# VladGavra98/SERL

Measured on AMD Instinct MI355X. Metric: env-steps/sec (whole node), pop-rollout eval, pop=50 nominal per GPU, higher is better.
Workload: dtype f64

## Files before the change

### serl_amd/csrc/citation_step_dev.h

```cpp
#if !defined(CIT_MODEL) || !defined(CIT_DERIV) || !defined(CIT_STEP)
#error "define CIT_MODEL, CIT_DERIV and CIT_STEP"
#endif
#ifndef CIT_STEP_ATTR
#define CIT_STEP_ATTR __noinline__
#endif
static __device__ CIT_STEP_ATTR void CIT_STEP(CitCtx *gc, const double *cmd_in, double *out_arg)
{
  CitCtx lc;
#ifdef CIT_CMD_IN_MEMORY
  double y[19], f[6][19], out[12];
#else
  double y[19], f[6][19], cmd[10], out[12];
#endif
  for (int i = 0; i < 19; ++i) { lc.X[i] = gc->X[i]; y[i] = lc.X[i]; }
#ifdef CIT_DW_IN_MEMORY
  lc.dwm = gc->DW;
#else
  for (int i = 0; i < 29; ++i) lc.DW[i] = gc->DW[i];
#endif
  for (int i = 0; i < 4; ++i) lc.IW[i] = gc->IW[i];
#ifndef CIT_Y_IS_STATE
  for (int i = 0; i < 12; ++i) lc.Y[i] = gc->Y[i];
#endif
#ifdef CIT_USE_HINTS
  for (int i = 0; i < (CIT_USE_HINTS + 5) / 6; ++i) lc.hint[i] = gc->hint[i];
#endif
#ifdef CIT_CMD_IN_MEMORY
  const double *cmd = cmd_in;
#else
  for (int i = 0; i < 10; ++i) cmd[i] = cmd_in[i];
#endif
  lc.t = gc->t; lc.stop_time = gc->stop_time; lc.dt = gc->dt; lc.tick = gc->tick;
  lc.ro = gc->ro; lc.t3 = gc->t3; lc.err = gc->err; lc.bslot = gc->bslot;
  const double t0 = lc.t, h = lc.dt;
  for (int s = 0; s < 6; ++s) {
    if (s > 0) {
      double hB[6];
      for (int j = 0; j < s; ++j) hB[j] = cit_ode5_B[s - 1][j] * h;
      for (int i = 0; i < 19; ++i) {
        double acc = f[0][i] * hB[0];
        for (int j = 1; j < s; ++j) acc = acc + f[j][i] * hB[j];
        lc.X[i] = acc + y[i];
      }
      lc.t = (s == 5) ? lc.stop_time : (s == 1 ? hB[0] + t0 : h * cit_ode5_A[s - 1] + t0);
    }
    lc.major = (s == 0) ? 1 : 0;
#ifndef CIT_NO_AXES
    cit_axes_prepare(&lc.ax, lc.X[4], lc.X[5], lc.X[6], lc.X[7], lc.X[8]);
#endif
    CIT_MODEL(&lc, cmd, out);
    CIT_DERIV(&lc, f[s]);
  }
  {
    double hB[6];
    for (int j = 0; j < 6; ++j) hB[j] = cit_ode5_B[5][j] * h;
    for (int i = 0; i < 19; ++i) {
      double acc = f[0][i] * hB[0];
      for (int j = 1; j < 6; ++j) acc = acc + f[j][i] * hB[j];
      gc->X[i] = acc + y[i];
    }
  }
#ifndef CIT_DW_IN_MEMORY
  for (int i = 0; i < 29; ++i) gc->DW[i] = lc.DW[i];
#endif
  for (int i = 0; i < 4; ++i) gc->IW[i] = lc.IW[i];
#ifdef CIT_Y_IS_STATE
  for (int i = 0; i < 12; ++i) { gc->Y[i] = y[i]; out_arg[i] = y[i]; }
#else
  for (int i = 0; i < 12; ++i) { gc->Y[i] = lc.Y[i]; out_arg[i] = lc.Y[i]; }
#endif
#ifdef CIT_USE_HINTS
  for (int i = 0; i < (CIT_USE_HINTS + 5) / 6; ++i) gc->hint[i] = lc.hint[i];
#endif
  gc->major = 1;
  gc->err = lc.err;
  gc->tick = lc.tick + 1;
  gc->stop_time = lc.stop_time;
  gc->t = lc.stop_time;
}
#undef CIT_MODEL
#undef CIT_DERIV
#undef CIT_STEP
#undef CIT_USE_HINTS
#undef CIT_Y_IS_STATE
#undef CIT_DW_IN_MEMORY
#undef CIT_CMD_IN_MEMORY
```

### serl_amd/csrc/family_lane.hip

```cpp
#include "citation_dev.h"
#include "rollout_device.h"
#include "serl_variant.h"
#ifdef SERL_VENV_NOISE
#include "serl_rng.h"
#endif
#ifdef SERL_ROLLOUT_NOISE
#include "rollout_noise.h"
#endif
#define CIT_V(x) SERL_PASTE(SERL_PASTE(cit_, VARIANT), x)
#define CIT_RO_LO_W CIT_V(_RO_LO_W)
#define CIT_RO_HI_W CIT_V(_RO_HI_W)
#define RO_BASE_W CIT_V(_RO_BASE_W)

namespace bdag {
#define CIT_B_AT(i) (c->B[(i)])
#define SERL_FLAVOUR_LDS 0
#define CIT_NO_AXES 1
#ifndef CIT_CTX_FLAT
#define CIT_DWM_PTR __attribute__((address_space(5))) double *
#define CIT_CMD_PTR const __attribute__((address_space(5))) double *
#else
#define CIT_DWM_PTR double *
#define CIT_CMD_PTR const double *
#endif
#include SERL_GEN_LANE
static_assert(CIT_RO_HI_W - CIT_RO_LO_W <= CIT_RO_LDS_WORDS, "LDS table window too small");
static_assert(8 * (CIT_RO_LDS_WORDS + CIT_V(_NSLOPE)) <= 160 * 1024, "tables + interval quotients beyond the 160 KB of LDS");
#define CIT_MODEL CIT_V(_dag_model)
#define CIT_DERIV CIT_V(_dag_derivatives)
#define CIT_STEP SERL_PASTE(cit_step_, VARIANT)
#define CIT_SLOPE_DESC CIT_V(_slope_desc)
#define CIT_SLOPE_TABLES CIT_V(_NSLOPE_TABLES)
#define CIT_USE_HINTS CIT_V(_NSEARCH)
#define CIT_DW_IN_MEMORY 1
#ifdef CIT_WITH_CMD_IN_MEMORY
#define CIT_CMD_IN_MEMORY 1
#endif
#if !defined(SERL_ROLLOUT_NOISE) && !defined(SERL_LANE_GENERAL_ACTOR)
#define SERL_LANE_QUEUE 1
#endif
#define CIT_Y_IS_STATE 1
#include "citation_step_dev.h"
#include "rollout_variant.inc"
#if !defined(SERL_ROLLOUT_NOISE) && !defined(SERL_LANE_GENERAL_ACTOR)
#include "venv_variant.inc"
#endif
#undef CIT_NO_AXES
#undef CIT_B_AT
#undef SERL_FLAVOUR_LDS
}

#define SERL_V(x) SERL_PASTE(x, VARIANT)
#if defined(SERL_LANE_GENERAL_ACTOR) && defined(SERL_LANE_REGROUPED_WEIGHTS)
#ifdef SERL_ROLLOUT_NOISE
void SERL_V(serl_launch_rollout_lanegt_noise_)(const RolloutArgs &a, const serl_rollout_noise_desc &nz, int grid, hipStream_t stream) { bdag::SERL_V(serl_launch_rollout_lanegt_noise_)(a, nz, grid, stream); }
#else
void SERL_V(serl_launch_rollout_lanegt_)(const RolloutArgs &a, int grid, hipStream_t stream) { bdag::SERL_V(serl_launch_rollout_lanegt_)(a, grid, stream); }
#endif
#elif defined(SERL_LANE_GENERAL_ACTOR)
#ifdef SERL_ROLLOUT_NOISE
void SERL_V(serl_launch_rollout_laneg_noise_)(const RolloutArgs &a, const serl_rollout_noise_desc &nz, int grid, hipStream_t stream) { bdag::SERL_V(serl_launch_rollout_laneg_noise_)(a, nz, grid, stream); }
#else
void SERL_V(serl_launch_rollout_laneg_)(const RolloutArgs &a, int grid, hipStream_t stream) { bdag::SERL_V(serl_launch_rollout_laneg_)(a, grid, stream); }
#endif
#elif defined(SERL_ROLLOUT_NOISE)
void SERL_V(serl_launch_rollout_noise_)(const RolloutArgs &a, const serl_rollout_noise_desc &nz, int grid, hipStream_t stream) { bdag::SERL_V(serl_launch_rollout_noise_)(a, nz, grid, stream); }
#elif defined(SERL_VENV_NOISE)
#define SERL_VNZ(x) SERL_PASTE(SERL_PASTE(x, noise_), VARIANT)
void SERL_VNZ(serl_launch_venv_reset_)(const RolloutArgs &a, const VenvArgs &v, const serl_venv_noise_desc &nz, int grid, hipStream_t stream) { bdag::SERL_VNZ(serl_launch_venv_reset_)(a, v, nz, grid, stream); }
void SERL_VNZ(serl_launch_venv_step_auto_)(const RolloutArgs &a, const VenvArgs &v, const serl_venv_auto_desc &au, const serl_venv_noise_desc &nz, int grid, hipStream_t stream) { bdag::SERL_VNZ(serl_launch_venv_step_auto_)(a, v, au, nz, grid, stream); }
void SERL_VNZ(serl_launch_venv_rollout_)(const RolloutArgs &a, const VenvArgs &v, const serl_venv_auto_desc &au, const serl_venv_rollout_desc &rd, const serl_venv_noise_desc &nz, int grid, hipStream_t stream) { bdag::SERL_VNZ(serl_launch_venv_rollout_)(a, v, au, rd, nz, grid, stream); }
void SERL_VNZ(serl_launch_venv_rollout_general_)(const RolloutArgs &a, const VenvArgs &v, const serl_venv_auto_desc &au, const serl_venv_rollout_desc &rd, const serl_venv_noise_desc &nz, int grid, hipStream_t stream) { bdag::SERL_VNZ(serl_launch_venv_rollout_general_)(a, v, au, rd, nz, grid, stream); }
#else
void SERL_V(serl_launch_rollout_)(const RolloutArgs &a, int grid, hipStream_t stream) { bdag::SERL_V(serl_launch_rollout_)(a, grid, stream); }
void SERL_V(serl_launch_rollout_laneq_)(const RolloutArgs &a, int grid, hipStream_t stream) { bdag::SERL_V(serl_launch_rollout_laneq_)(a, grid, stream); }

void SERL_V(serl_launch_dyn_)(const RolloutArgs &a, const double *cmds, double *states, int T, int grid, hipStream_t stream)
{
  bdag::SERL_V(serl_launch_dyn_)(a, cmds, states, T, grid, stream);
}

void SERL_V(serl_launch_venv_reset_)(const RolloutArgs &a, const VenvArgs &v, int grid, hipStream_t stream) { bdag::SERL_V(serl_launch_venv_reset_)(a, v, grid, stream); }
void SERL_V(serl_launch_venv_step_)(const RolloutArgs &a, const VenvArgs &v, int grid, hipStream_t stream) { bdag::SERL_V(serl_launch_venv_step_)(a, v, grid, stream); }
void SERL_V(serl_launch_venv_step_auto_)(const RolloutArgs &a, const VenvArgs &v, const serl_venv_auto_desc &au, int grid, hipStream_t stream) { bdag::SERL_V(serl_launch_venv_step_auto_)(a, v, au, grid, stream); }
void SERL_V(serl_launch_venv_rollout_)(const RolloutArgs &a, const VenvArgs &v, const serl_venv_auto_desc &au, const serl_venv_rollout_desc &rd, int grid, hipStream_t stream) { bdag::SERL_V(serl_launch_venv_rollout_)(a, v, au, rd, grid, stream); }
void SERL_V(serl_launch_venv_rollout_general_)(const RolloutArgs &a, const VenvArgs &v, const serl_venv_auto_desc &au, const serl_venv_rollout_desc &rd, int grid, hipStream_t stream) { bdag::SERL_V(serl_launch_venv_rollout_general_)(a, v, au, rd, grid, stream); }
#endif
```

### serl_amd/csrc/gen/citation_cg_timed_lane.inc

```
enum { cit_cg_timed_RO_BASE_W = 9216, cit_cg_timed_RO_LO_W = 9914, cit_cg_timed_RO_HI_W = 21883 };
enum { cit_cg_timed_NSEARCH = 47 };
enum { cit_cg_timed_NSLOPE = 8435, cit_cg_timed_NSLOPE_TABLES = 70 };
__shared__ double g_sl[cit_cg_timed_NSLOPE];
static __device__ const int cit_cg_timed_slope_desc[70][6] = {
  {1, 5091, 2, 1, 5089, 0},
  {1, 11914, 2, 1, 11912, 1},
  {1, 3085, 3, 1, 3082, 2},
  {1, 5590, 3, 1, 3088, 4},
  {1, 6444, 3, 1, 3088, 6},
  {1, 8405, 3, 1, 3088, 8},
  {1, 8408, 3, 1, 3088, 10},
  {1, 8414, 3, 1, 8411, 12},
  {1, 8414, 3, 1, 8417, 14},
  {1, 10200, 3, 1, 3088, 16},
  {2, 2594, 2, 2, 2590, 18},
  {2, 3103, 2, 2, 2590, 20},
  {2, 3131, 2, 2, 2590, 22},
  {2, 3131, 2, 2, 4115, 24},
  {2, 3135, 2, 2, 2590, 26},
  {2, 3139, 2, 2, 2590, 28},
  {2, 3143, 2, 2, 2590, 30},
  {2, 4117, 2, 2, 4115, 32},
  {2, 5577, 2, 2, 2590, 34},
  {2, 6255, 2, 2, 2590, 36},
  {2, 6261, 2, 2, 2590, 38},
  {2, 6346, 2, 2, 4115, 40},
  {2, 6350, 2, 2, 2590, 42},
  {2, 8424, 2, 2, 8420, 44},
  {2, 10213, 2, 2, 2590, 46},
  {2, 10404, 2, 2, 2590, 48},
  {2, 10498, 2, 2, 2590, 50},
  {1, 11920, 4, 1, 11916, 52},
  {1, 11907, 5, 1, 11902, 55},
  {1, 11924, 5, 1, 11902, 59},
  {1, 11896, 6, 1, 11890, 63},
  {2, 3094, 3, 3, 3088, 68},
  {2, 5581, 3, 3, 3088, 74},
  {2, 6147, 3, 3, 3088, 80},
  {2, 6435, 3, 3, 3088, 86},
  {2, 10191, 3, 3, 3088, 92},
  {2, 10314, 3, 3, 3088, 98},
  {2, 10408, 3, 3, 3088, 104},
  {1, 132, 10, 1, 122, 110},
  {1, 5593, 10, 1, 122, 119},
  {1, 10203, 10, 1, 122, 128},
  {2, 3115, 4, 4, 3107, 137},
  {2, 10298, 4, 4, 3107, 149},
  {2, 1744, 6, 6, 1732, 161},
  {2, 6174, 9, 9, 6156, 191},
  {2, 6265, 9, 9, 6156, 263},
  {2, 6354, 9, 9, 6156, 335},
  {2, 10217, 9, 9, 6156, 407},
  {2, 10323, 9, 9, 6156, 479},
  {2, 10417, 9, 9, 6156, 551},
  {2, 11614, 9, 9, 11596, 623},
  {2, 11469, 11, 11, 11447, 695},
  {2, 11721, 13, 13, 11695, 805},
  {2, 1814, 17, 17, 1780, 961},
  {2, 8428, 17, 17, 1780, 1233},
  {2, 214, 22, 22, 170, 1505},
  {2, 756, 22, 22, 734, 1967},
  {2, 1248, 22, 22, 734, 2429},
  {2, 2106, 22, 22, 734, 2891},
  {2, 2598, 22, 22, 734, 3353},
  {2, 3147, 22, 22, 170, 3815},
  {2, 3631, 22, 22, 734, 4277},
  {2, 4121, 22, 22, 734, 4739},
  {2, 4605, 22, 22, 734, 5201},
  {2, 5093, 22, 22, 734, 5663},
  {2, 5606, 22, 22, 734, 6125},
  {2, 6447, 22, 22, 170, 6587},
  {2, 6931, 22, 22, 734, 7049},
  {2, 7437, 22, 22, 7415, 7511},
  {2, 7921, 22, 22, 734, 7973},
};
static __device__ __forceinline__ double cit_table3_val(CitCtx *c, double u0, double u1, double u2)
{
  double y; cit_table3(c, &u0, &u1, &u2, &y); return y;
}
LIFT_INLINE void cit_cg_timed_dag_model(CitCtx *c, const double *cmd, double *out)
{
  (void)out;
  const double *X = c->X;
  const bool major = c->major != 0;
// ... 1338 lines not shown
```

### serl_amd/csrc/gen/citation_gust_lane.inc

```
enum { cit_gust_RO_BASE_W = 9216, cit_gust_RO_LO_W = 9914, cit_gust_RO_HI_W = 21888 };
enum { cit_gust_NSEARCH = 46 };
enum { cit_gust_NSLOPE = 8435, cit_gust_NSLOPE_TABLES = 70 };
__shared__ double g_sl[cit_gust_NSLOPE];
static __device__ const int cit_gust_slope_desc[70][6] = {
  {1, 5075, 2, 1, 5073, 0},
  {1, 11898, 2, 1, 11896, 1},
  {1, 3069, 3, 1, 3066, 2},
  {1, 5574, 3, 1, 3072, 4},
  {1, 6428, 3, 1, 3072, 6},
  {1, 8389, 3, 1, 3072, 8},
  {1, 8392, 3, 1, 3072, 10},
  {1, 8398, 3, 1, 8395, 12},
  {1, 8398, 3, 1, 8401, 14},
  {1, 10184, 3, 1, 3072, 16},
  {2, 2578, 2, 2, 2574, 18},
  {2, 3087, 2, 2, 2574, 20},
  {2, 3115, 2, 2, 2574, 22},
  {2, 3115, 2, 2, 4099, 24},
  {2, 3119, 2, 2, 2574, 26},
  {2, 3123, 2, 2, 2574, 28},
  {2, 3127, 2, 2, 2574, 30},
  {2, 4101, 2, 2, 4099, 32},
  {2, 5561, 2, 2, 2574, 34},
  {2, 6239, 2, 2, 2574, 36},
  {2, 6245, 2, 2, 2574, 38},
  {2, 6330, 2, 2, 4099, 40},
  {2, 6334, 2, 2, 2574, 42},
  {2, 8408, 2, 2, 8404, 44},
  {2, 10197, 2, 2, 2574, 46},
  {2, 10388, 2, 2, 2574, 48},
  {2, 10482, 2, 2, 2574, 50},
  {1, 11904, 4, 1, 11900, 52},
  {1, 11891, 5, 1, 11886, 55},
  {1, 11908, 5, 1, 11886, 59},
  {1, 11880, 6, 1, 11874, 63},
  {2, 3078, 3, 3, 3072, 68},
  {2, 5565, 3, 3, 3072, 74},
  {2, 6131, 3, 3, 3072, 80},
  {2, 6419, 3, 3, 3072, 86},
  {2, 10175, 3, 3, 3072, 92},
  {2, 10298, 3, 3, 3072, 98},
  {2, 10392, 3, 3, 3072, 104},
  {1, 132, 10, 1, 122, 110},
  {1, 5577, 10, 1, 122, 119},
  {1, 10187, 10, 1, 122, 128},
  {2, 3099, 4, 4, 3091, 137},
  {2, 10282, 4, 4, 3091, 149},
  {2, 1728, 6, 6, 1716, 161},
  {2, 6158, 9, 9, 6140, 191},
  {2, 6249, 9, 9, 6140, 263},
  {2, 6338, 9, 9, 6140, 335},
  {2, 10201, 9, 9, 6140, 407},
  {2, 10307, 9, 9, 6140, 479},
  {2, 10401, 9, 9, 6140, 551},
  {2, 11598, 9, 9, 11580, 623},
  {2, 11453, 11, 11, 11431, 695},
  {2, 11705, 13, 13, 11679, 805},
  {2, 1798, 17, 17, 1764, 961},
  {2, 8412, 17, 17, 1764, 1233},
  {2, 198, 22, 22, 154, 1505},
  {2, 740, 22, 22, 718, 1967},
  {2, 1232, 22, 22, 718, 2429},
  {2, 2090, 22, 22, 718, 2891},
  {2, 2582, 22, 22, 718, 3353},
  {2, 3131, 22, 22, 154, 3815},
  {2, 3615, 22, 22, 718, 4277},
  {2, 4105, 22, 22, 718, 4739},
  {2, 4589, 22, 22, 718, 5201},
  {2, 5077, 22, 22, 718, 5663},
  {2, 5590, 22, 22, 718, 6125},
  {2, 6431, 22, 22, 154, 6587},
  {2, 6915, 22, 22, 718, 7049},
  {2, 7421, 22, 22, 7399, 7511},
  {2, 7905, 22, 22, 718, 7973},
};
static __device__ __forceinline__ double cit_table3_val(CitCtx *c, double u0, double u1, double u2)
{
  double y; cit_table3(c, &u0, &u1, &u2, &y); return y;
}
LIFT_INLINE void cit_gust_dag_model(CitCtx *c, const double *cmd, double *out)
{
  (void)out;
  const double *X = c->X;
  const bool major = c->major != 0;
// ... 1335 lines not shown
```

### serl_amd/csrc/gen/citation_ice_lane.inc

```
enum { cit_ice_RO_BASE_W = 9216, cit_ice_RO_LO_W = 9914, cit_ice_RO_HI_W = 21888 };
enum { cit_ice_NSEARCH = 46 };
enum { cit_ice_NSLOPE = 8435, cit_ice_NSLOPE_TABLES = 70 };
__shared__ double g_sl[cit_ice_NSLOPE];
static __device__ const int cit_ice_slope_desc[70][6] = {
  {1, 5075, 2, 1, 5073, 0},
  {1, 11898, 2, 1, 11896, 1},
  {1, 3069, 3, 1, 3066, 2},
  {1, 5574, 3, 1, 3072, 4},
  {1, 6428, 3, 1, 3072, 6},
  {1, 8389, 3, 1, 3072, 8},
  {1, 8392, 3, 1, 3072, 10},
  {1, 8398, 3, 1, 8395, 12},
  {1, 8398, 3, 1, 8401, 14},
  {1, 10184, 3, 1, 3072, 16},
  {2, 2578, 2, 2, 2574, 18},
  {2, 3087, 2, 2, 2574, 20},
  {2, 3115, 2, 2, 2574, 22},
  {2, 3115, 2, 2, 4099, 24},
  {2, 3119, 2, 2, 2574, 26},
  {2, 3123, 2, 2, 2574, 28},
  {2, 3127, 2, 2, 2574, 30},
  {2, 4101, 2, 2, 4099, 32},
  {2, 5561, 2, 2, 2574, 34},
  {2, 6239, 2, 2, 2574, 36},
  {2, 6245, 2, 2, 2574, 38},
  {2, 6330, 2, 2, 4099, 40},
  {2, 6334, 2, 2, 2574, 42},
  {2, 8408, 2, 2, 8404, 44},
  {2, 10197, 2, 2, 2574, 46},
  {2, 10388, 2, 2, 2574, 48},
  {2, 10482, 2, 2, 2574, 50},
  {1, 11904, 4, 1, 11900, 52},
  {1, 11891, 5, 1, 11886, 55},
  {1, 11908, 5, 1, 11886, 59},
  {1, 11880, 6, 1, 11874, 63},
  {2, 3078, 3, 3, 3072, 68},
  {2, 5565, 3, 3, 3072, 74},
  {2, 6131, 3, 3, 3072, 80},
  {2, 6419, 3, 3, 3072, 86},
  {2, 10175, 3, 3, 3072, 92},
  {2, 10298, 3, 3, 3072, 98},
  {2, 10392, 3, 3, 3072, 104},
  {1, 132, 10, 1, 122, 110},
  {1, 5577, 10, 1, 122, 119},
  {1, 10187, 10, 1, 122, 128},
  {2, 3099, 4, 4, 3091, 137},
  {2, 10282, 4, 4, 3091, 149},
  {2, 1728, 6, 6, 1716, 161},
  {2, 6158, 9, 9, 6140, 191},
  {2, 6249, 9, 9, 6140, 263},
  {2, 6338, 9, 9, 6140, 335},
  {2, 10201, 9, 9, 6140, 407},
  {2, 10307, 9, 9, 6140, 479},
  {2, 10401, 9, 9, 6140, 551},
  {2, 11598, 9, 9, 11580, 623},
  {2, 11453, 11, 11, 11431, 695},
  {2, 11705, 13, 13, 11679, 805},
  {2, 1798, 17, 17, 1764, 961},
  {2, 8412, 17, 17, 1764, 1233},
  {2, 198, 22, 22, 154, 1505},
  {2, 740, 22, 22, 718, 1967},
  {2, 1232, 22, 22, 718, 2429},
  {2, 2090, 22, 22, 718, 2891},
  {2, 2582, 22, 22, 718, 3353},
  {2, 3131, 22, 22, 154, 3815},
  {2, 3615, 22, 22, 718, 4277},
  {2, 4105, 22, 22, 718, 4739},
  {2, 4589, 22, 22, 718, 5201},
  {2, 5077, 22, 22, 718, 5663},
  {2, 5590, 22, 22, 718, 6125},
  {2, 6431, 22, 22, 154, 6587},
  {2, 6915, 22, 22, 718, 7049},
  {2, 7421, 22, 22, 7399, 7511},
  {2, 7905, 22, 22, 718, 7973},
};
static __device__ __forceinline__ double cit_table3_val(CitCtx *c, double u0, double u1, double u2)
{
  double y; cit_table3(c, &u0, &u1, &u2, &y); return y;
}
LIFT_INLINE void cit_ice_dag_model(CitCtx *c, const double *cmd, double *out)
{
  (void)out;
  const double *X = c->X;
  const bool major = c->major != 0;
// ... 1332 lines not shown
```

### serl_amd/csrc/gen/citation_nominal_lane.inc

```
enum { cit_nominal_RO_BASE_W = 9216, cit_nominal_RO_LO_W = 9914, cit_nominal_RO_HI_W = 21884 };
enum { cit_nominal_NSEARCH = 46 };
enum { cit_nominal_NSLOPE = 8435, cit_nominal_NSLOPE_TABLES = 70 };
__shared__ double g_sl[cit_nominal_NSLOPE];
static __device__ const int cit_nominal_slope_desc[70][6] = {
  {1, 5071, 2, 1, 5069, 0},
  {1, 11894, 2, 1, 11892, 1},
  {1, 3065, 3, 1, 3062, 2},
  {1, 5570, 3, 1, 3068, 4},
  {1, 6424, 3, 1, 3068, 6},
  {1, 8385, 3, 1, 3068, 8},
  {1, 8388, 3, 1, 3068, 10},
  {1, 8394, 3, 1, 8391, 12},
  {1, 8394, 3, 1, 8397, 14},
  {1, 10180, 3, 1, 3068, 16},
  {2, 2574, 2, 2, 2570, 18},
  {2, 3083, 2, 2, 2570, 20},
  {2, 3111, 2, 2, 2570, 22},
  {2, 3111, 2, 2, 4095, 24},
  {2, 3115, 2, 2, 2570, 26},
  {2, 3119, 2, 2, 2570, 28},
  {2, 3123, 2, 2, 2570, 30},
  {2, 4097, 2, 2, 4095, 32},
  {2, 5557, 2, 2, 2570, 34},
  {2, 6235, 2, 2, 2570, 36},
  {2, 6241, 2, 2, 2570, 38},
  {2, 6326, 2, 2, 4095, 40},
  {2, 6330, 2, 2, 2570, 42},
  {2, 8404, 2, 2, 8400, 44},
  {2, 10193, 2, 2, 2570, 46},
  {2, 10384, 2, 2, 2570, 48},
  {2, 10478, 2, 2, 2570, 50},
  {1, 11900, 4, 1, 11896, 52},
  {1, 11887, 5, 1, 11882, 55},
  {1, 11904, 5, 1, 11882, 59},
  {1, 11876, 6, 1, 11870, 63},
  {2, 3074, 3, 3, 3068, 68},
  {2, 5561, 3, 3, 3068, 74},
  {2, 6127, 3, 3, 3068, 80},
  {2, 6415, 3, 3, 3068, 86},
  {2, 10171, 3, 3, 3068, 92},
  {2, 10294, 3, 3, 3068, 98},
  {2, 10388, 3, 3, 3068, 104},
  {1, 128, 10, 1, 118, 110},
  {1, 5573, 10, 1, 118, 119},
  {1, 10183, 10, 1, 118, 128},
  {2, 3095, 4, 4, 3087, 137},
  {2, 10278, 4, 4, 3087, 149},
  {2, 1724, 6, 6, 1712, 161},
  {2, 6154, 9, 9, 6136, 191},
  {2, 6245, 9, 9, 6136, 263},
  {2, 6334, 9, 9, 6136, 335},
  {2, 10197, 9, 9, 6136, 407},
  {2, 10303, 9, 9, 6136, 479},
  {2, 10397, 9, 9, 6136, 551},
  {2, 11594, 9, 9, 11576, 623},
  {2, 11449, 11, 11, 11427, 695},
  {2, 11701, 13, 13, 11675, 805},
  {2, 1794, 17, 17, 1760, 961},
  {2, 8408, 17, 17, 1760, 1233},
  {2, 194, 22, 22, 150, 1505},
  {2, 736, 22, 22, 714, 1967},
  {2, 1228, 22, 22, 714, 2429},
  {2, 2086, 22, 22, 714, 2891},
  {2, 2578, 22, 22, 714, 3353},
  {2, 3127, 22, 22, 150, 3815},
  {2, 3611, 22, 22, 714, 4277},
  {2, 4101, 22, 22, 714, 4739},
  {2, 4585, 22, 22, 714, 5201},
  {2, 5073, 22, 22, 714, 5663},
  {2, 5586, 22, 22, 714, 6125},
  {2, 6427, 22, 22, 150, 6587},
  {2, 6911, 22, 22, 714, 7049},
  {2, 7417, 22, 22, 7395, 7511},
  {2, 7901, 22, 22, 714, 7973},
};
static __device__ __forceinline__ double cit_table3_val(CitCtx *c, double u0, double u1, double u2)
{
  double y; cit_table3(c, &u0, &u1, &u2, &y); return y;
}
LIFT_INLINE void cit_nominal_dag_model(CitCtx *c, const double *cmd, double *out)
{
  (void)out;
  const double *X = c->X;
  const bool major = c->major != 0;
// ... 1327 lines not shown
```

### serl_amd/csrc/gen/citation_test_lane.inc

```
enum { cit_test_RO_BASE_W = 9216, cit_test_RO_LO_W = 9914, cit_test_RO_HI_W = 21888 };
enum { cit_test_NSEARCH = 46 };
enum { cit_test_NSLOPE = 8435, cit_test_NSLOPE_TABLES = 70 };
__shared__ double g_sl[cit_test_NSLOPE];
static __device__ const int cit_test_slope_desc[70][6] = {
  {1, 5075, 2, 1, 5073, 0},
  {1, 11898, 2, 1, 11896, 1},
  {1, 3069, 3, 1, 3066, 2},
  {1, 5574, 3, 1, 3072, 4},
  {1, 6428, 3, 1, 3072, 6},
  {1, 8389, 3, 1, 3072, 8},
  {1, 8392, 3, 1, 3072, 10},
  {1, 8398, 3, 1, 8395, 12},
  {1, 8398, 3, 1, 8401, 14},
  {1, 10184, 3, 1, 3072, 16},
  {2, 2578, 2, 2, 2574, 18},
  {2, 3087, 2, 2, 2574, 20},
  {2, 3115, 2, 2, 2574, 22},
  {2, 3115, 2, 2, 4099, 24},
  {2, 3119, 2, 2, 2574, 26},
  {2, 3123, 2, 2, 2574, 28},
  {2, 3127, 2, 2, 2574, 30},
  {2, 4101, 2, 2, 4099, 32},
  {2, 5561, 2, 2, 2574, 34},
  {2, 6239, 2, 2, 2574, 36},
  {2, 6245, 2, 2, 2574, 38},
  {2, 6330, 2, 2, 4099, 40},
  {2, 6334, 2, 2, 2574, 42},
  {2, 8408, 2, 2, 8404, 44},
  {2, 10197, 2, 2, 2574, 46},
  {2, 10388, 2, 2, 2574, 48},
  {2, 10482, 2, 2, 2574, 50},
  {1, 11904, 4, 1, 11900, 52},
  {1, 11891, 5, 1, 11886, 55},
  {1, 11908, 5, 1, 11886, 59},
  {1, 11880, 6, 1, 11874, 63},
  {2, 3078, 3, 3, 3072, 68},
  {2, 5565, 3, 3, 3072, 74},
  {2, 6131, 3, 3, 3072, 80},
  {2, 6419, 3, 3, 3072, 86},
  {2, 10175, 3, 3, 3072, 92},
  {2, 10298, 3, 3, 3072, 98},
  {2, 10392, 3, 3, 3072, 104},
  {1, 132, 10, 1, 122, 110},
  {1, 5577, 10, 1, 122, 119},
  {1, 10187, 10, 1, 122, 128},
  {2, 3099, 4, 4, 3091, 137},
  {2, 10282, 4, 4, 3091, 149},
  {2, 1728, 6, 6, 1716, 161},
  {2, 6158, 9, 9, 6140, 191},
  {2, 6249, 9, 9, 6140, 263},
  {2, 6338, 9, 9, 6140, 335},
  {2, 10201, 9, 9, 6140, 407},
  {2, 10307, 9, 9, 6140, 479},
  {2, 10401, 9, 9, 6140, 551},
  {2, 11598, 9, 9, 11580, 623},
  {2, 11453, 11, 11, 11431, 695},
  {2, 11705, 13, 13, 11679, 805},
  {2, 1798, 17, 17, 1764, 961},
  {2, 8412, 17, 17, 1764, 1233},
  {2, 198, 22, 22, 154, 1505},
  {2, 740, 22, 22, 718, 1967},
  {2, 1232, 22, 22, 718, 2429},
  {2, 2090, 22, 22, 718, 2891},
  {2, 2582, 22, 22, 718, 3353},
  {2, 3131, 22, 22, 154, 3815},
  {2, 3615, 22, 22, 718, 4277},
  {2, 4105, 22, 22, 718, 4739},
  {2, 4589, 22, 22, 718, 5201},
  {2, 5077, 22, 22, 718, 5663},
  {2, 5590, 22, 22, 718, 6125},
  {2, 6431, 22, 22, 154, 6587},
  {2, 6915, 22, 22, 718, 7049},
  {2, 7421, 22, 22, 7399, 7511},
  {2, 7905, 22, 22, 718, 7973},
};
static __device__ __forceinline__ double cit_table3_val(CitCtx *c, double u0, double u1, double u2)
{
  double y; cit_table3(c, &u0, &u1, &u2, &y); return y;
}
LIFT_INLINE void cit_test_dag_model(CitCtx *c, const double *cmd, double *out)
{
  (void)out;
  const double *X = c->X;
  const bool major = c->major != 0;
// ... 1335 lines not shown
```

### serl_amd/csrc/rollout_variant.inc

```
#define V_PASTE2(a, b) a##b
#define V_PASTE(a, b) V_PASTE2(a, b)
#define V_NAME(x) V_PASTE(x, VARIANT)

#ifndef SERL_VENV_NOISE
#ifdef SERL_ROLLOUT_NOISE
static __device__ void V_NAME(serl_wave_episodes_)(const RolloutArgs &a, const serl_rollout_noise_desc &nz, int e, bool active)
#else
static __device__ void V_NAME(serl_wave_episodes_)(const RolloutArgs &a, int e, bool active)
#endif
{
  const serl_rollout_desc &d = a.d;
  const int lane = threadIdx.x & 63;
  const double PI = 3.14159265358979323846;
  const double deg2rad = PI / 180.0, rad2deg = 180.0 / PI;
  const double bound = 10.0 * deg2rad, low = -bound, high = bound;
  const double max_theta = 60.0 * deg2rad, max_phi = 75.0 * deg2rad;
  const double scaler[3] = {6.0 / PI * 1.0, 6.0 / PI * 1.0, 6.0 / PI * 4.0};
  const double dt = 0.01;
  serl_fault_row f = {1.0, __longlong_as_double(0x7ff0000000000000LL), __longlong_as_double(0x7ff0000000000000LL),
                      0.0, 0.0, 0, 0, 0};
  const float *w = d.weights;
  const double *ref = d.ref;
  const serl_ref_spec *rspec = nullptr;
  const double *noise = nullptr;
// ... 31 lines not shown
    for (int i = 0; i < 10; ++i) cmd[i] = 0.0;
    cmd[0] = serl_clip(cmd[0] * f.elev_gain, -f.elev_clip, f.elev_clip);
    cmd[1] = serl_clip(cmd[1], -f.ail_clip, f.ail_clip);
    if (f.rudder_jam_on != 0.0) cmd[2] = f.rudder_jam;
    V_NAME(cit_step_)(&ctx, cmd, x);
    if (snoise) {
      const double *sn = snoise;
      x[0] += sn[0]; x[1] += sn[1]; x[2] += sn[2]; x[4] += sn[3]; x[5] += sn[4]; x[6] += sn[5]; x[7] += sn[6];
    }
#ifdef SERL_ROLLOUT_NOISE
    if (nzk.sensor) serl_rollout_noise_sensor(nz, nzk, 0, x);
#endif
    V0 = x[3];
    if (d.err0) for (int i = 0; i < 3; ++i) err[i] = d.err0[(size_t)e * 3 + i];
    obs[0] = err[0]; obs[1] = err[1]; obs[2] = err[2];
    obs[3] = x[0]; obs[4] = x[1]; obs[5] = x[2]; obs[6] = x[4];
  }

  const bool prof = a.prof != nullptr && blockIdx.x == 0 && threadIdx.x < 64;
  unsigned long long pc_actor = 0, pc_dyn = 0, pc_env = 0, pc_steps = 0, tc0 = 0, tc1 = 0, tc2 = 0;
#ifndef SERL_LANE_GENERAL_ACTOR
  const bool lane_actor = __builtin_amdgcn_readfirstlane((int)serl_lane_actor_ok(d)) != 0;
#endif
  for (;;) {
    const unsigned long long live = __ballot(!done);
    if (live == 0ULL) break;
    if (prof) tc0 = __builtin_readcyclecounter();
#ifdef SERL_LANE_GENERAL_ACTOR
    float act[3] = {0.0f, 0.0f, 0.0f};
    if (!done) {
      float obs16[16];
#pragma unroll
      for (int i = 0; i < 16; ++i) obs16[i] = i < 7 ? (float)obs[i] : 0.0f;
#ifdef SERL_LANE_REGROUPED_WEIGHTS
      serl_actor_forward_lane_general_t(d, a.wt, a.wt_members, member, obs16, act);
#else
      serl_actor_forward_lane_general(d, w, obs16, act);
#endif
    }
#else
    float obsf[7], act[3] = {0.0f, 0.0f, 0.0f};
    for (int i = 0; i < 7; ++i) obsf[i] = (float)obs[i];
    const unsigned wlo = (unsigned)(uintptr_t)w, whi = (unsigned)((uintptr_t)w >> 32);
    if (lane_actor) {
      if (a.wt) serl_actor_forward_lane32_t(d, a.wt, a.wt_members, member, obsf, act);
      else serl_actor_forward_lane32(d, w, obsf, act);
    } else
    for (int l = 0; l < a.lanes; ++l) {
      if (!((live >> l) & 1ULL)) continue;
      float o[7], r[3];
      for (int i = 0; i < 7; ++i) o[i] = serl_bcast(obsf[i], l);
      const uintptr_t wp = (uintptr_t)(unsigned)__builtin_amdgcn_readlane((int)wlo, l) |
                           ((uintptr_t)(unsigned)__builtin_amdgcn_readlane((int)whi, l) << 32);
      serl_actor_forward_wave(d, (const float *)wp, o, r);
      if (lane == l) { act[0] = r[0]; act[1] = r[1]; act[2] = r[2]; }
    }
#endif
    if (prof) { tc1 = __builtin_readcyclecounter(); pc_actor += tc1 - tc0; }
    if (done) continue;
    double u[3];
#ifdef SERL_ROLLOUT_NOISE
    if (nzk.action) {
      double dn[3];
      serl_rollout_noise_action(nz, nzk, k, dn);
      for (int i = 0; i < 3; ++i) {
        double an = serl_clip((double)act[i] + dn[i], -1.0, 1.0);
        u[i] = low + 0.5 * (an + 1.0) * (high - low);
        act[i] = (float)an;
      }
    } else
#endif
    if (noise) {
      for (int i = 0; i < 3; ++i) {
        double an = serl_clip((double)act[i] + noise[(size_t)k * 3 + i], -1.0, 1.0);
        u[i] = low + 0.5 * (an + 1.0) * (high - low);
        act[i] = (float)an;
      }
    } else {
      for (int i = 0; i < 3; ++i) {
        float s = 0.5f * (act[i] + 1.0f);
        u[i] = low + (double)s * (high - low);
      }
    }
    for (int i = 0; i < 10; ++i) cmd[i] = 0.0;
    cmd[0] = serl_clip(u[0] * f.elev_gain, -f.elev_clip, f.elev_clip);
    cmd[1] = serl_clip(u[1], -f.ail_clip, f.ail_clip);
    cmd[2] = (f.rudder_jam_on != 0.0) ? f.rudder_jam : u[2];
    V_NAME(cit_step_)(&ctx, cmd, x);
    if (snoise) {
      const double *sn = snoise + (size_t)(k + 1) * 7;
      x[0] += sn[0]; x[1] += sn[1]; x[2] += sn[2]; x[4] += sn[3]; x[5] += sn[4]; x[6] += sn[5]; x[7] += sn[6];
    }
#ifdef SERL_ROLLOUT_NOISE
    if (nzk.sensor) serl_rollout_noise_sensor(nz, nzk, k + 1, x);
#endif
    if (prof) { tc2 = __builtin_readcyclecounter(); pc_dyn += tc2 - tc1; }
    double rk[3];
    if (rspec) serl_ref_generate(rspec, t, d.t_max, rk[0], rk[1], rk[2]);
    else { rk[0] = ref[(size_t)k * 3]; rk[1] = ref[(size_t)k * 3 + 1]; rk[2] = ref[(size_t)k * 3 + 2]; }
    err[0] = rk[0] - x[7]; err[1] = rk[1] - x[6]; err[2] = rk[2] - x[5];
    double rsum = 0.0;
    for (int i = 0; i < 3; ++i) rsum = rsum + fabs(serl_clip(scaler[i] * err[i], -1.0, 1.0));
    double reward = -rsum / 3.0;
    int cost = (rad2deg * fabs(x[4]) > 11.0) || (rad2deg * fabs(x[6]) > 0.75 * max_phi) || (x[3] < V0 / 3.0);
    double nobs[7] = {err[0], err[1], err[2], x[0], x[1], x[2], x[4]};
    bool fin = (t >= d.t_max) || (fabs(x[7]) > max_theta) || (fabs(x[6]) > max_phi) || (x[9] < 50.0);
    if (fin) reward += -1.0 / dt * (d.t_max - t) * 2.0;
    t += dt;
    if (d.actions) for (int i = 0; i < 3; ++i) d.actions[((size_t)e * d.max_steps + k) * 3 + i] = u[i];
    if (d.states) for (int i = 0; i < 12; ++i) d.states[((size_t)e * d.max_steps + k) * 12 + i] = x[i];
    if (d.rewards) d.rewards[(size_t)e * d.max_steps + k] = reward;
    if (d.transitions) {
      float *tr = d.transitions + ((size_t)e * d.max_steps + k) * 20;
      for (int i = 0; i < 7; ++i) tr[i] = (float)obs[i];
      for (int i = 0; i < 3; ++i) tr[7 + i] = act[i];
      for (int i = 0; i < 7; ++i) tr[10 + i] = (float)nobs[i];
      tr[17] = (float)reward; tr[18] = fin ? 1.0f : 0.0f; tr[19] = cost ? 1.0f : 0.0f;
    }
    fitness += reward;
    cost_steps += cost;
    for (int i = 0; i < 7; ++i) obs[i] = nobs[i];
    ++k;
    if (prof) { pc_env += __builtin_readcyclecounter() - tc2; pc_steps += 1; }
    if (fin || k >= d.max_steps) {
      done = true;
      d.fitness[e] = fitness;
      d.length_steps[e] = fin ? k : -k;
      d.length_t[e] = t;
      d.cost_steps[e] = ctx.err ? -(1 << 30) : cost_steps;
    }
  }
  if (prof && lane == 0) { a.prof[0] = pc_actor; a.prof[1] = pc_dyn; a.prof[2] = pc_env; a.prof[3] = pc_steps; }
}

#ifdef SERL_LANE_QUEUE
static __device__ void V_NAME(serl_wave_episodes_q_)(const RolloutArgs &a, const int slot)
{
  const serl_rollout_desc &d = a.d;
  const int lane = threadIdx.x & 63;
  const double PI = 3.14159265358979323846;
  const double deg2rad = PI / 180.0, rad2deg = 180.0 / PI;
  const double bound = 10.0 * deg2rad, low = -bound, high = bound;
  const double max_theta = 60.0 * deg2rad, max_phi = 75.0 * deg2rad;
  const double scaler[3] = {6.0 / PI * 1.0, 6.0 / PI * 1.0, 6.0 / PI * 4.0};
  const double dt = 0.01;
  serl_fault_row f = {1.0, __longlong_as_double(0x7ff0000000000000LL), __longlong_as_double(0x7ff0000000000000LL),
                      0.0, 0.0, 0, 0, 0};
  const float *w = d.weights;
  const double *ref = d.ref;
  const serl_ref_spec *rspec = nullptr;
  const double *noise = nullptr;
  const double *snoise = nullptr;
  CitCtx ctx;
  double cmd[10], x[12], err[3] = {0, 0, 0}, obs[7] = {0, 0, 0, 0, 0, 0, 0};
  double V0 = 0.0, t = 0.0, fitness = 0.0;
  int k = 0, cost_steps = 0, e = slot;
  unsigned member = 0;
  bool retired = slot < 0;
  bool take = !retired;
  bool fresh = false;

  const bool lane_actor = __builtin_amdgcn_readfirstlane((int)serl_lane_actor_ok(d)) != 0;
  for (;;) {
    if (__ballot(!retired) == 0ULL) break;
    if (take) {
      f = serl_fault_row{1.0, __longlong_as_double(0x7ff0000000000000LL), __longlong_as_double(0x7ff0000000000000LL), 0.0, 0.0, 0, 0, 0};
      if (d.faults) f = d.faults[e];
      member = (unsigned)d.member_of_episode[e];
      w = d.weights + (size_t)member * d.weight_stride;
      ref = d.ref ? d.ref + (size_t)e * d.ref_stride : nullptr;
      rspec = d.ref_spec ? d.ref_spec + (size_t)e * d.ref_spec_stride : nullptr;
      snoise = nullptr; noise = nullptr;
      if (d.sensor_noise) {
        const int sr = d.sensor_row ? d.sensor_row[e] : e;
        if (sr >= 0) snoise = d.sensor_noise + (size_t)sr * ((size_t)d.max_steps + 1) * 7;
      }
      if (d.action_noise) {
        const int nr = d.noise_row ? d.noise_row[e] : e;
        if (nr >= 0) noise = d.action_noise + (size_t)nr * d.max_steps * 3;
      }
      cit_reset(&ctx, a.ro, a.t3, a.x0, a.dw0, a.dyn_dt);
      if (d.tick0) { ctx.tick = (uint32_t)d.tick0[e]; ctx.t = (double)ctx.tick * ctx.dt; }
      ctx.bslot = SERL_FLAVOUR_LDS ? ((threadIdx.x >> 6) * SERL_LDS_B_LANES_PER_WAVE + lane) * CIT_MAX_NB : 0;
      for (int i = 0; i < 3; ++i) err[i] = d.err0 ? d.err0[(size_t)e * 3 + i] : 0.0;
      t = 0.0; fitness = 0.0; k = 0; cost_steps = 0;
      take = false; fresh = true;
    }
    const unsigned long long flying = __ballot(!retired && !fresh);
    float obsf[7], act[3] = {0.0f, 0.0f, 0.0f};
    for (int i = 0; i < 7; ++i) obsf[i] = (float)obs[i];
    const unsigned wlo = (unsigned)(uintptr_t)w, whi = (unsigned)((uintptr_t)w >> 32);
    if (lane_actor) {
      if (a.wt) serl_actor_forward_lane32_t(d, a.wt, a.wt_members, member, obsf, act);
      else serl_actor_forward_lane32(d, w, obsf, act);
    } else
    for (int l = 0; l < a.lanes; ++l) {
      if (!((flying >> l) & 1ULL)) continue;
// ... 195 lines not shown
```

Measured before the change: 11.06 million.

## Accumulate Dormand-Prince stage sums on the fly instead of storing stage derivatives

Replaces the six-stage RK5 update, which keeps all stage derivatives f[6][19] and recombines them at each stage, with running per-stage accumulators. Each stage's derivative is added into the pending sums as soon as the model produces it, and states 13 and 14, whose derivative is statically zero, are skipped. The aim is to cut live registers or scratch and redundant multiply-adds in the lane kernel. The rollout loop also moves the action store and the observation float conversion before the dynamics step, shortening live ranges across the heavy call. The cost is an acc[6][17] array and a change in floating-point summation order, which is guarded to keep the zero terms.

```diff
diff --git a/serl_amd/csrc/citation_step_dev.h b/serl_amd/csrc/citation_step_dev.h
--- a/serl_amd/csrc/citation_step_dev.h
+++ b/serl_amd/csrc/citation_step_dev.h
@@ -33,6 +33,45 @@
   lc.t = gc->t; lc.stop_time = gc->stop_time; lc.dt = gc->dt; lc.tick = gc->tick;
   lc.ro = gc->ro; lc.t3 = gc->t3; lc.err = gc->err; lc.bslot = gc->bslot;
   const double t0 = lc.t, h = lc.dt;
+#ifdef CIT_ODE5_RUNNING
+  static_assert(CIT_XDOT_CONST_ZERO == 1, "states 13 and 14 must have the literal derivative +0");
+  double acc[6][17];
+  for (int s = 0; s < 6; ++s) {
+    if (s > 0) lc.t = (s == 5) ? lc.stop_time : (s == 1 ? cit_ode5_B[0][0] * h + t0 : h * cit_ode5_A[s - 1] + t0);
+    lc.major = (s == 0) ? 1 : 0;
+    CIT_MODEL(&lc, cmd, out);
+    double xn[19];
+    {
+      const double hb = cit_ode5_B[s][s] * h;
+      double zc = 0.0 * (cit_ode5_B[s][0] * h);
+      for (int j = 1; j <= s; ++j) zc = zc + 0.0 * (cit_ode5_B[s][j] * h);
+      if (s == 0) {
+#pragma unroll
+        for (int i = 0; i < 19; ++i) xn[i] = (i == 13 || i == 14) ? zc + y[i] : lc.B[i] * hb + y[i];
+      } else {
+#pragma unroll
+        for (int i = 0; i < 19; ++i) xn[i] = (i == 13 || i == 14) ? zc + y[i] : (acc[s][i < 13 ? i : i - 2] + lc.B[i] * hb) + y[i];
+      }
+    }
+    for (int r = s + 1; r < 6; ++r) {
+      const double hb = cit_ode5_B[r][s] * h;
+      if (s == 0) {
+#pragma unroll
+        for (int i = 0; i < 19; ++i) if (i != 13 && i != 14) acc[r][i < 13 ? i : i - 2] = lc.B[i] * hb;
+      } else {
+        double a[17];
+#pragma unroll
+        for (int k = 0; k < 17; ++k) a[k] = acc[r][k];
+#pragma unroll
+        for (int i = 0; i < 19; ++i) if (i != 13 && i != 14) a[i < 13 ? i : i - 2] = a[i < 13 ? i : i - 2] + lc.B[i] * hb;
+#pragma unroll
+        for (int k = 0; k < 17; ++k) acc[r][k] = a[k];
+      }
+    }
+    if (s == 5) { for (int i = 0; i < 19; ++i) gc->X[i] = xn[i]; }
+    else { for (int i = 0; i < 19; ++i) lc.X[i] = xn[i]; }
+  }
+#else
   for (int s = 0; s < 6; ++s) {
     if (s > 0) {
       double hB[6];
@@ -60,6 +99,7 @@
       gc->X[i] = acc + y[i];
     }
   }
+#endif
 #ifndef CIT_DW_IN_MEMORY
   for (int i = 0; i < 29; ++i) gc->DW[i] = lc.DW[i];
 #endif
@@ -85,3 +125,5 @@
 #undef CIT_Y_IS_STATE
 #undef CIT_DW_IN_MEMORY
 #undef CIT_CMD_IN_MEMORY
+#undef CIT_ODE5_RUNNING
+#undef CIT_XDOT_CONST_ZERO
diff --git a/serl_amd/csrc/family_lane.hip b/serl_amd/csrc/family_lane.hip
--- a/serl_amd/csrc/family_lane.hip
+++ b/serl_amd/csrc/family_lane.hip
@@ -39,6 +39,8 @@
 #if !defined(SERL_ROLLOUT_NOISE) && !defined(SERL_LANE_GENERAL_ACTOR)
 #define SERL_LANE_QUEUE 1
 #endif
+#define CIT_ODE5_RUNNING 1
+#define CIT_XDOT_CONST_ZERO CIT_V(_XDOT_CONST_ZERO)
 #define CIT_Y_IS_STATE 1
 #include "citation_step_dev.h"
 #include "rollout_variant.inc"
diff --git a/serl_amd/csrc/gen/citation_cg_timed_lane.inc b/serl_amd/csrc/gen/citation_cg_timed_lane.inc
--- a/serl_amd/csrc/gen/citation_cg_timed_lane.inc
+++ b/serl_amd/csrc/gen/citation_cg_timed_lane.inc
@@ -1,5 +1,6 @@
 enum { cit_cg_timed_RO_BASE_W = 9216, cit_cg_timed_RO_LO_W = 9914, cit_cg_timed_RO_HI_W = 21883 };
 enum { cit_cg_timed_NSEARCH = 47 };
+enum { cit_cg_timed_XDOT_CONST_ZERO = 1 };
 enum { cit_cg_timed_NSLOPE = 8435, cit_cg_timed_NSLOPE_TABLES = 70 };
 __shared__ double g_sl[cit_cg_timed_NSLOPE];
 static __device__ const int cit_cg_timed_slope_desc[70][6] = {
diff --git a/serl_amd/csrc/gen/citation_gust_lane.inc b/serl_amd/csrc/gen/citation_gust_lane.inc
--- a/serl_amd/csrc/gen/citation_gust_lane.inc
+++ b/serl_amd/csrc/gen/citation_gust_lane.inc
@@ -1,5 +1,6 @@
 enum { cit_gust_RO_BASE_W = 9216, cit_gust_RO_LO_W = 9914, cit_gust_RO_HI_W = 21888 };
 enum { cit_gust_NSEARCH = 46 };
+enum { cit_gust_XDOT_CONST_ZERO = 1 };
 enum { cit_gust_NSLOPE = 8435, cit_gust_NSLOPE_TABLES = 70 };
 __shared__ double g_sl[cit_gust_NSLOPE];
 static __device__ const int cit_gust_slope_desc[70][6] = {
diff --git a/serl_amd/csrc/gen/citation_ice_lane.inc b/serl_amd/csrc/gen/citation_ice_lane.inc
--- a/serl_amd/csrc/gen/citation_ice_lane.inc
+++ b/serl_amd/csrc/gen/citation_ice_lane.inc
@@ -1,5 +1,6 @@
 enum { cit_ice_RO_BASE_W = 9216, cit_ice_RO_LO_W = 9914, cit_ice_RO_HI_W = 21888 };
 enum { cit_ice_NSEARCH = 46 };
+enum { cit_ice_XDOT_CONST_ZERO = 1 };
 enum { cit_ice_NSLOPE = 8435, cit_ice_NSLOPE_TABLES = 70 };
 __shared__ double g_sl[cit_ice_NSLOPE];
 static __device__ const int cit_ice_slope_desc[70][6] = {
diff --git a/serl_amd/csrc/gen/citation_nominal_lane.inc b/serl_amd/csrc/gen/citation_nominal_lane.inc
--- a/serl_amd/csrc/gen/citation_nominal_lane.inc
+++ b/serl_amd/csrc/gen/citation_nominal_lane.inc
@@ -1,5 +1,6 @@
 enum { cit_nominal_RO_BASE_W = 9216, cit_nominal_RO_LO_W = 9914, cit_nominal_RO_HI_W = 21884 };
 enum { cit_nominal_NSEARCH = 46 };
+enum { cit_nominal_XDOT_CONST_ZERO = 1 };
 enum { cit_nominal_NSLOPE = 8435, cit_nominal_NSLOPE_TABLES = 70 };
 __shared__ double g_sl[cit_nominal_NSLOPE];
 static __device__ const int cit_nominal_slope_desc[70][6] = {
diff --git a/serl_amd/csrc/gen/citation_test_lane.inc b/serl_amd/csrc/gen/citation_test_lane.inc
--- a/serl_amd/csrc/gen/citation_test_lane.inc
+++ b/serl_amd/csrc/gen/citation_test_lane.inc
@@ -1,5 +1,6 @@
 enum { cit_test_RO_BASE_W = 9216, cit_test_RO_LO_W = 9914, cit_test_RO_HI_W = 21888 };
 enum { cit_test_NSEARCH = 46 };
+enum { cit_test_XDOT_CONST_ZERO = 1 };
 enum { cit_test_NSLOPE = 8435, cit_test_NSLOPE_TABLES = 70 };
 __shared__ double g_sl[cit_test_NSLOPE];
 static __device__ const int cit_test_slope_desc[70][6] = {
diff --git a/serl_amd/csrc/rollout_variant.inc b/serl_amd/csrc/rollout_variant.inc
--- a/serl_amd/csrc/rollout_variant.inc
+++ b/serl_amd/csrc/rollout_variant.inc
@@ -137,6 +137,9 @@
         u[i] = low + (double)s * (high - low);
       }
     }
+    if (d.actions) for (int i = 0; i < 3; ++i) d.actions[((size_t)e * d.max_steps + k) * 3 + i] = u[i];
+    float tobs[7];
+    for (int i = 0; i < 7; ++i) tobs[i] = (float)obs[i];
     for (int i = 0; i < 10; ++i) cmd[i] = 0.0;
     cmd[0] = serl_clip(u[0] * f.elev_gain, -f.elev_clip, f.elev_clip);
     cmd[1] = serl_clip(u[1], -f.ail_clip, f.ail_clip);
@@ -162,12 +165,11 @@
     bool fin = (t >= d.t_max) || (fabs(x[7]) > max_theta) || (fabs(x[6]) > max_phi) || (x[9] < 50.0);
     if (fin) reward += -1.0 / dt * (d.t_max - t) * 2.0;
     t += dt;
-    if (d.actions) for (int i = 0; i < 3; ++i) d.actions[((size_t)e * d.max_steps + k) * 3 + i] = u[i];
     if (d.states) for (int i = 0; i < 12; ++i) d.states[((size_t)e * d.max_steps + k) * 12 + i] = x[i];
     if (d.rewards) d.rewards[(size_t)e * d.max_steps + k] = reward;
     if (d.transitions) {
       float *tr = d.transitions + ((size_t)e * d.max_steps + k) * 20;
-      for (int i = 0; i < 7; ++i) tr[i] = (float)obs[i];
+      for (int i = 0; i < 7; ++i) tr[i] = tobs[i];
       for (int i = 0; i < 3; ++i) tr[7 + i] = act[i];
       for (int i = 0; i < 7; ++i) tr[10 + i] = (float)nobs[i];
       tr[17] = (float)reward; tr[18] = fin ? 1.0f : 0.0f; tr[19] = cost ? 1.0f : 0.0f;
```

Result: no change. 11.08 million (median of 6 runs) (+0.1%).
